# lionelblonde/sac-td3-cudagraphs-pytorch

Hardware: AMD Instinct MI355X
Metric: gradient-steps/sec (SAC, batch=256) at 1 GPU + 8-seed node; replay HBM GB/s (higher is better)
Workload: dtype f32; 1 GPU; SAC Hopper-v4 batch=256 2x256 MLP+LN, 100000 rows in a 1000000-row HBM ring, 1 critic update+Polyak per iteration, 2 actor+alpha updates every 3rd, hipGraph per 3 iterations; parallelism=1 independent seeds, one per GPU, no collective

## Files before the change

### sac-td3-cudagraphs-pytorch_amd/csrc/engine.hip

```cpp
#include <hip/hip_runtime.h>

#include <algorithm>
#include <cmath>
#include <cstdio>
#include <cstdlib>
#include <cstring>
#include <string>
#include <chrono>
#include <vector>

#include "../../include/sactd3.h"
#include "kernels.h"

static thread_local std::string g_create_error;

static inline int round_up(int x, int m) { return (x + m - 1) / m * m; }
static inline unsigned magic_div(unsigned d, unsigned long long n_max) {
  return (d > 1 && n_max * d < (1ull << 32)) ? (unsigned)(((1ull << 32) + d - 1) / d) : 0u;
}

static NetLayout make_layout(int K, int nh) {
  NetLayout L{};
  L.K = K; L.ld1 = round_up(K, 4); L.nh = nh;
  int off = 0;
// ... 68 lines not shown
  float *la = nullptr, *gscale = nullptr;
  float* ring = nullptr; float* stage_dev = nullptr;
  float *X = nullptr, *Xn = nullptr, *Xp = nullptr, *rew = nullptr, *done = nullptr;
  int* idx = nullptr;
  float *logp_n = nullptr, *logp_pi = nullptr, *logp_al = nullptr, *act_scratch = nullptr;
  float* eps[SACTD3_NUM_SITES] = {};
  float *a_z1 = nullptr, *a_xh1 = nullptr, *a_h1 = nullptr, *a_rs1 = nullptr, *a_z2 = nullptr, *a_xh2 = nullptr, *a_h2 = nullptr, *a_rs2 = nullptr, *a_tg = nullptr;
  float *a_du = nullptr, *a_dz2 = nullptr, *a_dh1 = nullptr, *a_dz1 = nullptr;
  float *qa_ps = nullptr, *qa_S = nullptr;
  float *a_ps = nullptr, *c_ps = nullptr;
  float* a_z2n = nullptr;
  float* ah_z1[4] = {}; float* ah_z2[4] = {};
  struct BatchSlot { float *X, *Xn, *rew, *done, *logp_n, *eps_c; int* idx; } bs[4] = {};
  int cur_slot = 0;
  int chain_ready = -1;
  float *c_z1 = nullptr, *c_xh1 = nullptr, *c_h1 = nullptr, *c_rs1 = nullptr, *c_z2 = nullptr, *c_dz2 = nullptr, *c_dh1 = nullptr, *c_dz1 = nullptr;
  float *t_z1 = nullptr, *t_z2 = nullptr, *q = nullptr, *qt = nullptr, *y = nullptr, *q_pi = nullptr, *dA = nullptr;
  float* s_h1 = nullptr;
  float* Gp = nullptr; int gp_slabs = 0;
  float *part = nullptr, *part_s = nullptr, *part_sa = nullptr;
  float *p_x = nullptr, *p_z1 = nullptr, *p_z2 = nullptr, *p_act = nullptr;
  float *h_obs = nullptr, *h_act = nullptr;
  int* h_done = nullptr; int predict_calls = 0;
  float* h_stage[NSTAGE] = {}; int stage_next = 0, stage_used = 0;
  float* h_batch = nullptr;

  int64_t rb_len = 0, rb_cursor = 0, qnet_updates = 0;
  hipGraphExec_t graphs[G_COUNT] = {}; int graph_nodes[G_COUNT] = {};
  std::vector<hipGraphExec_t> predict_graphs;
  hipStream_t act_stream = nullptr;
// ... 223 lines not shown
    fl += 2.0 * nets * (double)g.M * q.N * q.K;
    by += 4.0 * nets * (double)g.M * (q.N + q.K);
  }
  a.tiles_per_net = tiles;
  const int nch = (g.M + TN64_M - 1) / TN64_M;
  int S = (2 * e->num_cus + tiles * nets / 2) / (tiles * nets);
  S = std::max(1, std::min(S, std::min(e->gp_slabs, nch)));
  a.S = S;
  const long size = a.g_ns;
  {
    const dim3 grid((unsigned)(tiles * nets * S));
    char inst[96];
    snprintf(inst, sizeof(inst), "k_tn64<2,2,2,1,64>.dW(split-M x%d)", S);
    LAUNCH(inst, fl, by + 4.0 * S * nets * (double)size, TN64_KERNEL, grid, dim3(256), a);
  }
  r.Gp = e->Gp; r.S = S; r.nets = nets; r.g_ns = size; r.G = g.G;
  r.apply = g.apply; r.P = g.P; r.Mo = g.Mo; r.Vo = g.Vo; r.T = g.T; r.tau = g.tau; r.adam = g.adam; r.b1 = g.b1; r.b2 = g.b2; r.eps = g.eps;
  r.part = g.part; r.pstride = g.pstride; r.part_s = g.part_s;
  r.loss_part = g.loss_part; r.loss_n = g.loss_n; r.loss_stride = g.loss_stride; r.loss_off = g.loss_off; r.loss_scale = g.loss_scale;
  r.loss_dst = g.loss_dst; r.tick = g.tick; r.tick_extra = tick_extra;
  const dim3 grid((unsigned)((size / 4 + 255) / 256 + 4 * r.nvec + 1), (unsigned)nets);
  LAUNCH(g.apply ? (g.T ? "k_adam_red.sum+adam+polyak" : "k_adam_red.sum+adam") : "k_adam_red.sum", 0.0,
         nets * (double)size * (4.0 * S + 4.0 + (g.apply ? 24.0 : 0.0) + (g.apply && g.T ? 8.0 : 0.0)), k_adam_red, grid, dim3(256), r);
  (void)name;
  return 0;
}

static inline int tn_width(const TnProb& q) { return q.kw > 0 ? q.kw : q.ldw; }
static int launch_tn(sactd3_engine* e, hipStream_t s, const char* name, TnArgs& g, int nets, int tick_extra = 0) {
  if (g.M >= BIG_BATCH && e->Gp && !e->tune_tn_kt) {
    int tiles = 0;
    for (int i = 0; i < g.nprob; ++i) tiles += ((g.pr[i].N + TN64_N - 1) / TN64_N) * ((g.pr[i].ldw + TN64_K - 1) / TN64_K);
    if (tiles * nets >= e->tune_tn64_min) return launch_tn64(e, s, name, g, nets, tick_extra);
  }
  auto count = [&](int kt) {
    int tiles = 0;
    for (int i = 0; i < g.nprob; ++i) {
      g.pr[i].tile0 = tiles;
      tiles += ((g.pr[i].N + 15) / 16) * (((tn_width(g.pr[i]) + 15) / 16 + kt - 1) / kt);
    }
    return tiles;
  };
  int kt = (count(1) * nets > 2 * e->num_cus && g.M < BIG_BATCH) ? 2 : 1;
  if (e->tune_tn_kt) kt = e->tune_tn_kt;
// ... 9 lines not shown
  bool fold = false;
  for (int i = 0; i < g.nprob; ++i) fold = fold || g.pr[i].fold;
  char inst[96];
  snprintf(inst, sizeof(inst), fold ? "k_tn<%d,true>.%s" : "k_tn<%d>.%s", kt, name);
  g.tiles = tiles;
  if (g.pk_blocks) by += 12.0 * (g.pk.n0 + g.pk.n1);
  {
    AdamRedArgs& r = g.fin;
    r = AdamRedArgs{};
    r.s_off = -1;
    for (int i = 0; i < g.nprob; ++i) {
      const TnProb& q = g.pr[i];
      for (int f = 0; f < q.nfin; ++f) { r.vec[r.nvec].off = q.fin_off[f]; r.vec[r.nvec].slot = q.fin_slot[f]; r.vec[r.nvec].nblk = q.fin_nblk[f]; ++r.nvec; }
      if (q.fin_s_off >= 0) { r.s_off = q.fin_s_off; r.s_nblk = q.fin_s_nblk; }
    }
    r.nets = nets; r.g_ns = g.g_ns; r.G = g.G;
    r.apply = g.apply; r.P = g.P; r.Mo = g.Mo; r.Vo = g.Vo; r.T = g.T; r.tau = g.tau; r.adam = g.adam; r.b1 = g.b1; r.b2 = g.b2; r.eps = g.eps;
    r.T2 = g.T2; r.T3 = g.T3;
    r.part = g.part; r.pstride = g.pstride; r.part_s = g.part_s;
    r.loss_part = g.loss_part; r.loss_n = g.loss_n; r.loss_stride = g.loss_stride; r.loss_off = g.loss_off; r.loss_scale = g.loss_scale;
    r.loss_dst = g.loss_dst; r.tick = g.tick; r.tick_extra = tick_extra;
    g.fin_blocks = 4 * r.nvec + 1;
  }
  const dim3 grid((unsigned)((tiles + g.pk_blocks + g.fin_blocks + (nets > 1 ? 7 : 0)) & (nets > 1 ? ~7 : ~0)), 1, (unsigned)nets);
  if (!node_on(e, inst, fl, by, grid, dim3(256))) return 0;
  if (fold) {
    if (kt == 2) hipLaunchKernelGGL((k_tn<2, true>), grid, dim3(256), 0, s, g);
    else hipLaunchKernelGGL((k_tn<1, true>), grid, dim3(256), 0, s, g);
  } else if (kt == 2) hipLaunchKernelGGL(k_tn<2>, grid, dim3(256), 0, s, g);
  else hipLaunchKernelGGL(k_tn<1>, grid, dim3(256), 0, s, g);
  HIPCHK(hipGetLastError());
  return 0;
}
static TnProb tn_prob(const float* dY, int ldy, long dy_ns, int N, const float* X, int ldx, long x_ns, int K,
                      int w_off, int ldw, int b_off) {
  TnProb q{};
  q.dY = dY; q.ldy = ldy; q.dy_ns = dy_ns; q.N = N; q.X = X; q.ldx = ldx; q.x_ns = x_ns; q.K = K;
  q.w_off = w_off; q.ldw = ldw; q.b_off = b_off; q.nfin = 0; q.fin_s_off = -1;
  return q;
}
static TnProb tn_rows(const TnProb& q, int n_lo, int n) {
  TnProb r = q;
  r.dY = q.dY + n_lo; r.N = n; r.w_off = q.w_off + n_lo * q.ldw; r.b_off = q.b_off >= 0 ? q.b_off + n_lo : -1;
  if (n_lo) { r.nfin = 0; r.fin_s_off = -1; r.x_dup = 1; }
  return r;
// ... 1157 lines not shown
int sactd3_read_noise(sactd3_engine* e, int site, float* eps, int n) {
  if (!e || !eps || site < 0 || site >= SACTD3_NUM_SITES || n < 1 || n > std::max(e->B, e->maxn)) return SACTD3_EINVAL;
  USE_DEVICE(e);
  if (e->act_inflight && site == SACTD3_SITE_PREDICT) return e->fail(SACTD3_ESTATE, "read_noise: an acting call is in flight (sactd3_predict_end first)");
  HIPCHK(hipStreamSynchronize(e->stream));
  const float* src = site == SACTD3_SITE_CRITIC ? e->bs[e->cur_slot].eps_c : e->eps[site];
  HIPCHK(hipMemcpy(eps, src, sizeof(float) * (size_t)n * e->a, hipMemcpyDeviceToHost));
  return 0;
}

int sactd3_update_qnets(sactd3_engine* e) {
  if (!e) return SACTD3_EINVAL;
  USE_DEVICE(e);
  CHAIN_BREAK(e);
  e->cur_slot = 0;
  return run_graph(e, G_Q, [&](hipStream_t s) { return enqueue_update_qnets(e, s, false, nullptr); });
}
int sactd3_update_actor(sactd3_engine* e) {
  if (!e) return SACTD3_EINVAL;
  USE_DEVICE(e);
  CHAIN_BREAK(e);
  RCCHK(actor_write_begin(e));
  return run_graph(e, G_A, [&](hipStream_t s) { return enqueue_update_actor(e, s, 0); });
}
int sactd3_update_targ_nets(sactd3_engine* e, int64_t qnet_updates_so_far) {
  if (!e) return SACTD3_EINVAL;
  USE_DEVICE(e);
  CHAIN_BREAK(e);
  const bool td3 = e->cfg.prefer_td3_over_sac;
  if (td3 || qnet_updates_so_far % e->cfg.crit_targ_update_freq == 0) return enqueue_polyak(e, e->stream, true, td3);
  return 0;
}
int sactd3_step(sactd3_engine* e, int do_actor) {
  if (!e) return SACTD3_EINVAL;
  USE_DEVICE(e);
  CHAIN_BREAK(e);
  if (e->rb_len <= 0) return e->fail(SACTD3_ESTATE, "step: buffer is empty");
  const int64_t updates = e->qnet_updates + 1;
  const bool polyak = e->cfg.prefer_td3_over_sac || (updates % e->cfg.crit_targ_update_freq == 0);
  const bool act = do_actor != 0 && e->cfg.actor_update_delay > 0;
  const int which = G_STEP00 + (act ? 2 : 0) + (polyak ? 1 : 0);
  if (act) RCCHK(actor_write_begin(e));
  RCCHK(run_graph(e, which, [&](hipStream_t s) { return enqueue_step(e, s, act, polyak); }));
  e->qnet_updates = updates;
  e->cur_slot = 0;
  return 0;
}

static bool actor_dw_is_tiled64(const sactd3_engine* e) {
  if (e->B < BIG_BATCH || !e->Gp || e->tune_tn_kt) return false;
  const int tiles = ((e->nh + TN64_N - 1) / TN64_N) * ((HID + TN64_K - 1) / TN64_K) + ((HID + TN64_N - 1) / TN64_N) * ((HID + TN64_K - 1) / TN64_K)
                    + ((HID + TN64_N - 1) / TN64_N) * ((e->La.ld1 + TN64_K - 1) / TN64_K);
  return tiles >= e->tune_tn64_min;
}
static bool period_is_pipelined(const sactd3_engine* e) {
  const sactd3_config& c = e->cfg;
  if (c.actor_update_delay < 1 || c.actor_update_delay > 2 || !opening_trunk_gathers(e)) return false;
  if (c.prefer_td3_over_sac) return c.clip_norm <= 0.f && !actor_dw_is_tiled64(e);
  return c.autotune != 0;
}
static int enqueue_period(sactd3_engine* e, hipStream_t s, int variant = 0) {
  const int n = e->cfg.actor_update_delay + 1;
  if (!period_is_pipelined(e)) {
    for (int i = 0; i < n; ++i) RCCHK(enqueue_step(e, s, i == 0 && e->cfg.actor_update_delay > 0, true, i + 1 < n));
  } else {
    const int P = variant ? 3 : 0, Pnext = variant ? 0 : 3;
    RCCHK(enqueue_step(e, s, true, true, true, P, true, n - 1, Pnext, true));
    for (int i = 1; i < n; ++i) RCCHK(enqueue_step(e, s, false, true, i + 1 < n, i, true));
  }
  if (e->alpha_pending) return e->fail(SACTD3_ESTATE, "step_period: a deferred temperature step was left over");
  return 0;
}
static int enqueue_prefix(sactd3_engine* e, hipStream_t s, int variant, int m) {
  const int P = variant ? 3 : 0;
  RCCHK(enqueue_step(e, s, true, true, m > 1, P, true, m - 1, -1, true));
  for (int i = 1; i < m; ++i) RCCHK(enqueue_step(e, s, false, true, i + 1 < m, i, true));
  if (e->alpha_pending) return e->fail(SACTD3_ESTATE, "step_prefix: a deferred temperature step was left over");
  return 0;
}
static int enqueue_opening(sactd3_engine* e, hipStream_t s, int slot) {
  bool policy_done = false;
  return enqueue_update_qnets(e, s, true, nullptr, true, &policy_done, false, nullptr, slot, false, 1);
}

int sactd3_step_period(sactd3_engine* e) {
  if (!e) return SACTD3_EINVAL;
  USE_DEVICE(e);
  if (e->rb_len <= 0) return e->fail(SACTD3_ESTATE, "step_period: buffer is empty");
  const bool td3 = e->cfg.prefer_td3_over_sac;
  if (!td3 && e->cfg.crit_targ_update_freq != 1) return e->fail(SACTD3_ESTATE, "step_period: needs crit_targ_update_freq == 1");
  const int n = e->cfg.actor_update_delay + 1;
  RCCHK(actor_write_begin(e));
  if (!period_is_pipelined(e)) {
    e->chain_ready = -1;
    RCCHK(run_graph(e, G_PERIOD, [&](hipStream_t s) { return enqueue_period(e, s); }));
    e->cur_slot = 0;
  } else {
    const int v = e->chain_ready >= 0 ? e->chain_ready : 0;
    const bool have = e->chain_ready >= 0;
    e->chain_ready = -1;
    if (!have) RCCHK(run_graph(e, G_OPENING, [&](hipStream_t s) { return enqueue_opening(e, s, 0); }));
    RCCHK(run_graph(e, v ? G_PERIOD_B : G_PERIOD, [&](hipStream_t s) { return enqueue_period(e, s, v); }));
    e->chain_ready = 1 - v;
    e->cur_slot = n - 1;
  }
  e->qnet_updates += n;
  return 0;
// ... 1 lines not shown

int sactd3_step_prefix(sactd3_engine* e, int m) {
  if (!e) return SACTD3_EINVAL;
  USE_DEVICE(e);
  if (m < 1 || m > e->cfg.actor_update_delay) return e->fail(SACTD3_EINVAL, "step_prefix: 1 <= m <= actor_update_delay");
  if (e->rb_len <= 0) return e->fail(SACTD3_ESTATE, "step_prefix: buffer is empty");
  if (!e->cfg.prefer_td3_over_sac && e->cfg.crit_targ_update_freq != 1) return e->fail(SACTD3_ESTATE, "step_prefix: needs crit_targ_update_freq == 1");
  if (!period_is_pipelined(e) || m > 2) {
    for (int i = 0; i < m; ++i) RCCHK(sactd3_step(e, i == 0));
    return 0;
  }
  const int v = e->chain_ready >= 0 ? e->chain_ready : 0;
  const bool have = e->chain_ready >= 0;
  e->chain_ready = -1;
  RCCHK(actor_write_begin(e));
  if (!have) RCCHK(run_graph(e, G_OPENING, [&](hipStream_t s) { return enqueue_opening(e, s, 0); }));
  RCCHK(run_graph(e, G_PREFIX + 2 * (m - 1) + v, [&](hipStream_t s) { return enqueue_prefix(e, s, v, m); }));
  e->cur_slot = m - 1;
  e->qnet_updates += m;
  return 0;
}

int sactd3_instantiate_graphs(sactd3_engine* e) {
  if (!e) return SACTD3_EINVAL;
  USE_DEVICE(e);
  const bool same_branch = e->cfg.prefer_td3_over_sac || e->cfg.crit_targ_update_freq == 1;
  for (int act = 0; act < 2; ++act)
    for (int pol = same_branch ? 1 : 0; pol < 2; ++pol) {
      const bool a = act != 0 && e->cfg.actor_update_delay > 0, py = pol != 0;
      RCCHK(run_graph(e, G_STEP00 + (a ? 2 : 0) + (py ? 1 : 0), [&](hipStream_t s) { return enqueue_step(e, s, a, py); }, false));
// ... 171 lines not shown
      {"logp_next", S.logp_n, B}, {"logp_pi", e->logp_pi, B}, {"logp_alpha", e->logp_al, B},
      {"a_xh1", e->a_xh1, BH}, {"a_h1", e->a_h1, BH}, {"a_z2", e->a_z2, BH}, {"a_h2", e->a_h2, BH}, {"a_du", e->a_du, B * e->ldu},
      {"a_dz2", e->a_dz2, BH}, {"a_dh1", e->a_dh1, BH}, {"a_dz1", e->a_dz1, BH},
      {"c_xh1", e->c_xh1, 2 * BH}, {"c_h1", e->c_h1, 2 * BH}, {"c_z2", e->c_z2, 2 * BH}, {"c_dz2", e->c_dz2, 2 * BH},
      {"c_dh1", e->c_dh1, 2 * BH}, {"c_dz1", e->c_dz1, 2 * BH}, {"t_z2", e->t_z2, 2 * BH},
      {"q", e->q, 2 * B}, {"q_target", e->qt, 2 * B}, {"targ_q", e->y, B}, {"q_pi", e->q_pi, 2 * B}, {"dA", e->dA, 2 * B * e->a4},
  };
}
const char* sactd3_debug_names(void) {
  return "X Xn Xp rew done logp_next logp_pi logp_alpha a_xh1 a_h1 a_z2 a_h2 a_du a_dz2 a_dh1 a_dz1 c_xh1 c_h1 c_z2 c_dz2 c_dh1 c_dz1 "
         "t_z2 q q_target targ_q q_pi dA grad_actor grad_critics";
}
int64_t sactd3_debug_read(sactd3_engine* e, const char* name, float* dst, int64_t max_floats) {
  if (!e || !name) return SACTD3_EINVAL;
  USE_DEVICE(e);
  if (!strcmp(name, "grad_actor") || !strcmp(name, "grad_critics")) {
    const bool act = !strcmp(name, "grad_actor");
    const int64_t n = sactd3_param_count(e, act ? SACTD3_ACTOR : SACTD3_CRITICS);
    if (!dst) return n;
    if (max_floats < n) return e->fail(SACTD3_EINVAL, "debug_read: buffer too small");
    RCCHK(read_arena(e, act ? e->Ga : e->Gc, act ? e->La : e->Lc, act ? 1 : 2, dst));
    return n;
  }
  for (const DbgEntry& d : dbg_table(e)) {
    if (strcmp(d.name, name)) continue;
    if (!dst) return d.n;
    if (max_floats < d.n) return e->fail(SACTD3_EINVAL, "debug_read: buffer too small");
    HIPCHK(hipStreamSynchronize(e->stream));
    HIPCHK(hipMemcpy(dst, d.ptr, sizeof(float) * d.n, hipMemcpyDeviceToHost));
    return d.n;
// ... 43 lines not shown
    *usec = ms * 1000.f / (float)iters;
  }
  hipEventDestroy(t0); hipEventDestroy(t1);
  return rc;
}

int sactd3_time_nodes(sactd3_engine* e, int do_actor, int iters, int max_nodes, char* names, int names_cap,
                      float* usec, double* flops, double* bytes, int64_t* threads) {
  if (!e || iters < 1 || max_nodes < 1 || !usec) return SACTD3_EINVAL;
  USE_DEVICE(e);
  CHAIN_BREAK(e);
  if (e->rb_len <= 0) return e->fail(SACTD3_ESTATE, "time_nodes: buffer is empty");
  const bool act = do_actor != 0 && e->cfg.actor_update_delay > 0;
  const bool period = do_actor == 2 && e->cfg.actor_update_delay > 0 && (e->cfg.prefer_td3_over_sac || e->cfg.crit_targ_update_freq == 1);
  if (act || period) RCCHK(actor_write_begin(e));
  std::vector<NodeInfo> log;
  auto seq = [&]() -> int { e->node_seq = 0; return period ? enqueue_period(e, e->stream) : enqueue_step(e, e->stream, act, true); };
  auto done = [&](int rc) { e->node_only = -1; e->node_log = nullptr; e->node_seq = 0; e->node_role = ""; return rc; };
  e->node_log = &log; e->node_only = 1 << 30;
  int rc = seq();
  e->node_log = nullptr;
  if (rc != 0) return done(rc);
  const int n = (int)log.size();
  if (n > max_nodes) return done(e->fail(SACTD3_EINVAL, "time_nodes: max_nodes too small"));
  std::string joined;
  for (int k = 0; k < n; ++k) { joined += log[k].name; joined += '\n'; }
  if (names) {
    if ((int)joined.size() + 1 > names_cap) return done(e->fail(SACTD3_EINVAL, "time_nodes: names buffer too small"));
    memcpy(names, joined.c_str(), joined.size() + 1);
  }
// ... 98 lines not shown
```

### sac-td3-cudagraphs-pytorch_amd/csrc/kernels.h

```cpp
#pragma once
#include <hip/hip_runtime.h>
#include <stddef.h>
#include <stdint.h>
#include <type_traits>
#include "philox.h"

#define HID 256
#define LN_EPS 1e-5f
#define NSLOT 5
#define AS 260
#define WS 68
#define YS 20

typedef float f32x4 __attribute__((ext_vector_type(4)));

#ifdef SACTD3_STAMPS
__device__ long long g_stamps[16];
__device__ long long g_phase[8];
#define PHASE_DECL long long ph_t = 0, ph_acc[6] = {0, 0, 0, 0, 0, 0}
#define PHASE_START do { __builtin_amdgcn_s_waitcnt(0xc07f); ph_t = clock64(); } while (0)
#define PHASE(i) do { const long long n_ = clock64(); ph_acc[i] += n_ - ph_t; ph_t = n_; } while (0)
#define PHASE_DRAIN(i) do { __builtin_amdgcn_s_waitcnt(0); const long long n_ = clock64(); ph_acc[i] += n_ - ph_t; ph_t = n_; } while (0)
#define PHASE_OUT do { if (threadIdx.x == 0 && blockIdx.x == gridDim.x - 1) for (int i_ = 0; i_ < 6; ++i_) g_phase[i_] = ph_acc[i_]; } while (0)
#define STAMP(i) do { if (threadIdx.x == 0 && blockIdx.x == gridDim.x - 1 && blockIdx.y == 0 && blockIdx.z == 0) { __builtin_amdgcn_s_waitcnt(0); g_stamps[i] = clock64(); } } while (0)
// ... 96 lines not shown
  v += dpp_mov<0x141>(v);
  v += dpp_mov<0x140>(v);
  return v;
}
__device__ __forceinline__ float lane_bcast(float v, int l) {
  return __builtin_bit_cast(float, __builtin_amdgcn_readlane(__builtin_bit_cast(int, v), l));
}
__device__ __forceinline__ float wave_sum(float v) {
  v = row16_sum(v);
  return (lane_bcast(v, 0) + lane_bcast(v, 16)) + (lane_bcast(v, 32) + lane_bcast(v, 48));
}
__device__ __forceinline__ float sum4(float4 v) { return (v.x + v.y) + (v.z + v.w); }
__device__ __forceinline__ float dot4(float4 a, float4 b) { return a.x * b.x + a.y * b.y + a.z * b.z + a.w * b.w; }
__device__ __forceinline__ float4 ld4(const float* p) { return *reinterpret_cast<const float4*>(p); }
__device__ __forceinline__ void st4(float* p, float4 v) { *reinterpret_cast<float4*>(p) = v; }
__device__ __forceinline__ float4 f4(float a) { return make_float4(a, a, a, a); }
__device__ __forceinline__ float4 operator+(float4 a, float4 b) { return make_float4(a.x + b.x, a.y + b.y, a.z + b.z, a.w + b.w); }
__device__ __forceinline__ float4 operator-(float4 a, float4 b) { return make_float4(a.x - b.x, a.y - b.y, a.z - b.z, a.w - b.w); }
__device__ __forceinline__ float4 operator*(float4 a, float4 b) { return make_float4(a.x * b.x, a.y * b.y, a.z * b.z, a.w * b.w); }
__device__ __forceinline__ float4 operator*(float4 a, float b) { return make_float4(a.x * b, a.y * b, a.z * b, a.w * b); }
__device__ __forceinline__ float4 relu4(float4 a) { return make_float4(fmaxf(a.x, 0.f), fmaxf(a.y, 0.f), fmaxf(a.z, 0.f), fmaxf(a.w, 0.f)); }
__device__ __forceinline__ float4 gate4(float4 v, float4 y) {
  return make_float4(y.x > 0.f ? v.x : 0.f, y.y > 0.f ? v.y : 0.f, y.z > 0.f ? v.z : 0.f, y.w > 0.f ? v.w : 0.f);
}
__device__ __forceinline__ float4 ld4_cols(const float* row, int k, int K, int Kr, bool row_ok = true) {
  const float4 v = ld4(row + min(k, Kr - 4));
  float4 o;
  o.x = (row_ok && k < K) ? v.x : 0.f;
  o.y = (row_ok && k + 1 < K) ? v.y : 0.f;
  o.z = (row_ok && k + 2 < K) ? v.z : 0.f;
// ... 474 lines not shown
  } else {
    __syncthreads();
    if (PRO == 2) {
#pragma unroll
      for (int c = 0; c < CW; ++c) { xh[c] = av[c]; av[c] = relu4(av[c]); }
    }
  }
  STAMP(2); BLK_PH_K(1, 2);
  if (PRO != 0 && m0 + r < p.M) {
    const long ro = ni * p.act_ns + (long)(m0 + r) * HID + kb;
    const int gsz = 16 / tiles_n, g0 = tn * gsz;
#pragma unroll
    for (int c = 0; c < CW; ++c) {
      const int gc = ks * CW + c;
      if (gc >= g0 && gc < g0 + gsz) {
        if (G.xh_out) st4(G.xh_out + ro + 16 * c, xh[c]);
        if (G.h_out) st4(G.h_out + ro + 16 * c, av[c]);
      }
    }
    if (G.rstd_out && tn == 0 && ks == 0 && kq == 0) G.rstd_out[(long)ni * p.M + m0 + r] = rstd;
  }
  constexpr int NH = C4 ? 2 : 1;
  f32x4 acc[NT], ph[NT][NH];
  {
    constexpr int GC = CW < 4 ? CW : 4;
#pragma unroll
    for (int h = 0; h < NH; ++h) {
      f32x4 a0[NT], a1[NT];
#pragma unroll
      for (int nt = 0; nt < NT; ++nt) { a0[nt] = f32x4{0.f, 0.f, 0.f, 0.f}; a1[nt] = f32x4{0.f, 0.f, 0.f, 0.f}; }
#pragma unroll
      for (int c0 = h * (CW / NH); c0 < (h + 1) * (CW / NH); c0 += GC) {
// ... 37 lines not shown
            const float4 o = ld4(red + (((nt * 4 + wave + j) * NH + h) * 64 + lane) * 4);
            acc[nt][0] += o.x; acc[nt][1] += o.y; acc[nt][2] += o.z; acc[nt][3] += o.w;
          }
    }
  }
  STAMP(4); BLK_PH_K(1, 4);
  if (ks == 0) {
    float* y = G.Y + ni * p.y_ns;
#pragma unroll
    for (int nt = 0; nt < NT; ++nt) {
      const int col = n0 + 16 * nt + (lane & 15);
      if (col >= p.N) continue;
#pragma unroll
      for (int i = 0; i < 4; ++i) {
        const int row = m0 + 4 * (lane >> 4) + i;
        if (row < p.M) y[(long)row * p.ldy + col] = acc[nt][i] + bias[nt];
      }
    }
  }
  STAMP(5); BLK_PH_K(1, 5);
  BLK_MARK_K(1, 1);
}

__global__ __launch_bounds__(256) void k_nt_wide(NtArgs p) {
  __shared__ __attribute__((aligned(16))) float red[4 * 64 * 4];
  const int t = threadIdx.x, lane = t & 63, wave = t >> 6, net = blockIdx.z;
  const int r = lane & 15, kq = lane >> 4;
  if (blockIdx.x == 0 && t == 0 && net == 0) {
    if (p.tick0 || p.tick1) tick_all(p.tick0, p.tick1, p.adam_pw, p.adam_out, p.lr, p.b1, p.b2);
  }
  if (blockIdx.x == 0 && t == 64 && net == 0 && p.tick0b) tick_all(p.tick0b, nullptr, p.adam_pw_b, p.adam_out_b, p.lr_b, p.b1, p.b2);
// ... 404 lines not shown
  float* x = p.dX + net * p.dx_ns;
#pragma unroll
  for (int tt = 0; tt < TT; ++tt) {
    const int col = n0 + 16 * TT * wn + 16 * tt + r;
#pragma unroll
    for (int i = 0; i < 4; ++i) {
      const int row = m0 + 16 * wm + 4 * kq + i;
      if (row < p.M) x[(long)row * p.ldx + col] = acc[tt][i];
    }
  }
}

struct AdamRedVec { int off; int slot; int nblk; };
struct AdamRedArgs {
  const float* Gp; int S; int nets; long g_ns;
  float* G;
  int apply; float* P; float* Mo; float* Vo; float* T; float tau;
  float* T2; float* T3;
  const float* adam; float b1, b2, eps;
  AdamRedVec vec[5]; int nvec;
  const float* part; int pstride;
  int s_off; int s_nblk; const float* part_s;
  const float* loss_part; int loss_n, loss_stride, loss_off; float loss_scale; float* loss_dst; int* tick;
  int tick_extra;
};
__device__ __forceinline__ void adam_red_commit(const AdamRedArgs& a, long off, float4 g, float4 w, float4 m, float4 v, float4 tt, float step, float sq2) {
  st4(a.G + off, g);
  if (a.apply) {
    const float omb1 = 1.0f - a.b1, omb2 = 1.0f - a.b2;
    m = m + (g - m) * omb1;
    v = v * a.b2 + g * g * omb2;
    w.x -= step * (m.x / (sqrtf(v.x) / sq2 + a.eps)); w.y -= step * (m.y / (sqrtf(v.y) / sq2 + a.eps));
    w.z -= step * (m.z / (sqrtf(v.z) / sq2 + a.eps)); w.w -= step * (m.w / (sqrtf(v.w) / sq2 + a.eps));
    st4(a.Mo + off, m); st4(a.Vo + off, v); st4(a.P + off, w);
    if (a.T) {
      const float4 t1 = tt + (w - tt) * a.tau;
      st4(a.T + off, t1);
      if (a.T2) {
        const float4 t2 = t1 + (w - t1) * a.tau;
        st4(a.T2 + off, t2);
        if (a.T3) st4(a.T3 + off, t2 + (w - t2) * a.tau);
      }
    }
  }
}
__device__ __forceinline__ void adam_red_tail_body(const AdamRedArgs& a, int rel, int net) {
  const int t = threadIdx.x;
  const float step = a.apply ? a.adam[0] : 0.f, sq2 = a.apply ? a.adam[1] : 1.f;
  if (rel < 4 * a.nvec) {
    const int e = rel >> 2, quarter = rel & 3;
    int voff = a.vec[0].off, vslot = a.vec[0].slot, nb = a.vec[0].nblk;
    if (e == 1) { voff = a.vec[1].off; vslot = a.vec[1].slot; nb = a.vec[1].nblk; }
    if (e == 2) { voff = a.vec[2].off; vslot = a.vec[2].slot; nb = a.vec[2].nblk; }
    if (e == 3) { voff = a.vec[3].off; vslot = a.vec[3].slot; nb = a.vec[3].nblk; }
    if (e == 4) { voff = a.vec[4].off; vslot = a.vec[4].slot; nb = a.vec[4].nblk; }
    const int c4 = (t >> 4) + 16 * quarter, sub = t & 15;
    const long off = net * a.g_ns + voff + 4 * c4;
    float4 w = f4(0.f), m = f4(0.f), v = f4(0.f), tt = f4(0.f);
    if (a.apply && sub == 0) { w = ld4(a.P + off); m = ld4(a.Mo + off); v = ld4(a.Vo + off); if (a.T) tt = ld4(a.T + off); }
    const float* pp = a.part + ((long)net * a.pstride * NSLOT + vslot) * HID + 4 * c4;
    float4 g = f4(0.f);
    for (int blk = sub; blk < nb; blk += 64) {
      const float4 v0 = ld4(pp + (long)blk * NSLOT * HID), v1 = ld4(pp + (long)min(blk + 16, nb - 1) * NSLOT * HID);
      const float4 v2 = ld4(pp + (long)min(blk + 32, nb - 1) * NSLOT * HID), v3 = ld4(pp + (long)min(blk + 48, nb - 1) * NSLOT * HID);
      g = g + v0;
      if (blk + 16 < nb) g = g + v1;
      if (blk + 32 < nb) g = g + v2;
      if (blk + 48 < nb) g = g + v3;
    }
    g.x = row16_sum(g.x); g.y = row16_sum(g.y); g.z = row16_sum(g.z); g.w = row16_sum(g.w);
    if (sub == 0) adam_red_commit(a, off, g, w, m, v, tt, step, sq2);
    return;
  }
  if (t >= 64) return;
  const bool extras = net == 0;
  float loss_acc = 0.f; int tick_v = 0;
  if (extras) {
    if (a.loss_dst) for (int k = t; k < a.loss_n; k += 64) loss_acc += a.loss_part[(long)k * a.loss_stride + a.loss_off];
    if (t == 0 && a.tick) tick_v = *a.tick;
  }
  if (a.s_off >= 0) {
    const long off = net * a.g_ns + a.s_off;
    float4 w = f4(0.f), m = f4(0.f), v = f4(0.f), tt = f4(0.f);
    if (a.apply && t == 0) { w = ld4(a.P + off); m = ld4(a.Mo + off); v = ld4(a.Vo + off); if (a.T) tt = ld4(a.T + off); }
    float sg = 0.f;
    for (int blk = t; blk < a.s_nblk; blk += 64) sg += a.part_s[((long)net * a.pstride + blk) * 2];
    sg = wave_sum(sg);
    if (t == 0) adam_red_commit(a, off, make_float4(sg, 0.f, 0.f, 0.f), w, m, v, tt, step, sq2);
  }
  if (extras) {
    if (a.loss_dst) {
      const float sl = wave_sum(loss_acc);
      if (t == 0) *a.loss_dst = sl * a.loss_scale;
    }
    if (t == 0 && a.tick) *a.tick = tick_v + 1 + a.tick_extra;
  }
}

struct PolyakArgs { float* t0; const float* p0; long n0; float* t1; const float* p1; long n1; float tau; };
__device__ __forceinline__ void polyak_body(const PolyakArgs& a, unsigned block, unsigned nblocks) {
  const long n = a.n0 + a.n1;
  for (long i = ((long)block * 256 + threadIdx.x) * 4; i < n; i += (long)nblocks * 1024) {
    float* t = i < a.n0 ? a.t0 + i : a.t1 + (i - a.n0);
// ... 11 lines not shown
  int nfin; int fin_slot[3]; int fin_off[3]; int fin_nblk[3];
  int fin_s_off; int fin_s_nblk;
  int tile0;
  int xr;
  int x_dup;
  int xr_force;
  int kw;
  int fold, f_ln, f_g_off, f_be_off;
  const float* f_xh; const float* f_rstd; const float* f_ps; float* f_dz;
  const float* f_g;
};
constexpr int PS_W = 32;
struct TnArgs {
  TnProb pr[4]; int nprob; int M;
  float* G; long g_ns;
  int apply; float* P; float* Mo; float* Vo; float* T; float tau; float* T2; float* T3;
  const float* adam;
  float b1, b2, eps;
  const float* part; int pstride; const float* part_s;
  const float* loss_part; int loss_n, loss_stride, loss_off; float loss_scale; float* loss_dst; int* tick;
  int tiles; int pk_blocks; PolyakArgs pk;
  int fin_blocks; AdamRedArgs fin;
};

struct AdamState { float w, m, v, t; };
__device__ __forceinline__ AdamState adam_fetch(const TnArgs& p, long off) {
  AdamState s{0.f, 0.f, 0.f, 0.f};
  if (p.apply) { s.w = p.P[off]; s.m = p.Mo[off]; s.v = p.Vo[off]; if (p.T) s.t = p.T[off]; }
  return s;
}
__device__ __forceinline__ void adam_commit(const TnArgs& p, long off, float g, AdamState s, float step, float sq2) {
  p.G[off] = g;
  if (p.apply) {
    const float m = s.m + (g - s.m) * (1.0f - p.b1);
    const float v = s.v * p.b2 + g * g * (1.0f - p.b2);
    const float w = s.w - step * (m / (sqrtf(v) / sq2 + p.eps));
    p.Mo[off] = m; p.Vo[off] = v; p.P[off] = w;
    if (p.T) {
      const float t1 = s.t + (w - s.t) * p.tau;
      p.T[off] = t1;
      if (p.T2) {
        const float t2 = t1 + (w - t1) * p.tau;
        p.T2[off] = t2;
        if (p.T3) p.T3[off] = t2 + (w - t2) * p.tau;
      }
    }
  }
}

template <int KT, bool FOLD = false>
__global__ __launch_bounds__(256) void k_tn(TnArgs p) {
  __shared__ __attribute__((aligned(16))) float red[KT * 4 * 64 * 4];
  __shared__ __attribute__((aligned(16))) float Ys[256 * YS];
  __shared__ __attribute__((aligned(16))) float Xs[KT * 256 * YS];
  __shared__ float cred[16 * 17];
  __shared__ __attribute__((aligned(16))) float fsum[FOLD ? 16 * 4 * 8 : 4];
  const int t = threadIdx.x, lane = t & 63, wave = t >> 6, net = blockIdx.z;
  const int r = lane & 15, kq = lane >> 4;
  BLK_MARK(0);
  if ((int)blockIdx.x >= p.tiles) {
    const int x = (int)blockIdx.x - p.tiles;
    if (x < p.pk_blocks) { if (net == 0) polyak_body(p.pk, x, p.pk_blocks); }
    else if (x - p.pk_blocks < p.fin_blocks) adam_red_tail_body(p.fin, x - p.pk_blocks, net);
    BLK_MARK(1);
    return;
  }
  int pi = 0;
  if (p.nprob > 1 && (int)blockIdx.x >= p.pr[1].tile0) pi = 1;
  if (p.nprob > 2 && (int)blockIdx.x >= p.pr[2].tile0) pi = 2;
  if (p.nprob > 3 && (int)blockIdx.x >= p.pr[3].tile0) pi = 3;
  const TnProb q = p.pr[pi];
  const int local = blockIdx.x - q.tile0;
  const int kw = q.kw > 0 ? q.kw : q.ldw;
  const int tiles_k = (((kw + 15) >> 4) + KT - 1) / KT;
  int tn, tk;
  xcd_tile(local, (q.N + 15) >> 4, tiles_k, q.xr, tn, tk);
  const int n0 = tn * 16, k0 = tk * 16 * KT;
  const long nbase = net * p.g_ns;
// ... 96 lines not shown
  STAMP(2); BLK_PH(2);
#pragma unroll
  for (int kt = 0; kt < KT; ++kt) st4(red + ((kt * 4 + wave) * 64 + lane) * 4, make_float4(acc[kt][0], acc[kt][1], acc[kt][2], acc[kt][3]));
  if (want_bias) cred[fpart * 17 + fcol] = asum;
  if (fold_vec) {
    float v[8] = {cg.x, cg.y, cg.z, cg.w, cb.x, cb.y, cb.z, cb.w};
#pragma unroll
    for (int j = 0; j < 8; ++j) { v[j] += dpp_mov<0x124>(v[j]); v[j] += dpp_mov<0x128>(v[j]); }
    if ((lane & 15) < 4) {
      float* d = fsum + ((wave * 4 + (lane >> 4)) * 4 + (lane & 3)) * 8;
      st4(d, make_float4(v[0], v[1], v[2], v[3])); st4(d + 4, make_float4(v[4], v[5], v[6], v[7]));
    }
  }
  __syncthreads();
  STAMP(3); BLK_PH(3);
  if (wave < KT && ecol < kw) {
    const float* rr = red + (wave * 4 * 64 + lane) * 4;
    const float4 a = ld4(rr), b = ld4(rr + 256), c = ld4(rr + 512), d = ld4(rr + 768);
    const float o[4] = {(a.x + b.x) + (c.x + d.x), (a.y + b.y) + (c.y + d.y), (a.z + b.z) + (c.z + d.z), (a.w + b.w) + (c.w + d.w)};
#pragma unroll
    for (int i = 0; i < 4; ++i) {
      const int row = n0 + 4 * (lane >> 4) + i;
      if (row < q.N) adam_commit(p, nbase + q.w_off + (long)row * q.ldw + ecol, ecol < q.K ? o[i] : 0.f, st[i], step, sq2);
    }
  }
  if (foff >= 0) {
    float v = 0.f;
    if (lane < 16) {
#pragma unroll
      for (int i = 0; i < 16; ++i) v += cred[i * 17 + fcol];
    } else {
      const float* f = fsum + (fcol >> 2) * 8 + (lane < 32 ? 0 : 4) + (fcol & 3);
#pragma unroll
      for (int i = 0; i < 16; ++i) v += f[i * 32];
    }
    adam_commit(p, foff, v, fstate, step, sq2);
  }
  STAMP(4); BLK_PH(4);
  BLK_MARK(1);
}

struct Tn64Prob {
  const float* dY; int ldy; long dy_ns; int N;
  const float* X; int ldx; long x_ns; int K;
  int w_off, ldw, b_off;
  int tiles_n, tiles_k, tile0;
};
struct Tn64Args {
  Tn64Prob pr[3]; int nprob; int M; int nets; int S;
  int tiles_per_net;
  float* Gp; long g_ns;
// ... 162 lines not shown
  }
  if (want_bias) {
    constexpr int PARTS = 256 / TN;
    csum[t] = asum;
    __syncthreads();
    if (t < TN && n0 + t < q.N) {
      float v = 0.f;
#pragma unroll
      for (int i = 0; i < PARTS; ++i) v += csum[i * TN + t];
      Gs[q.b_off + n0 + t] = v;
    }
  }
  STAMP(3);
}

__global__ __launch_bounds__(256) void k_adam_red(AdamRedArgs a) {
  const int net = blockIdx.y, t = threadIdx.x;
  const int main_blocks = (int)((a.g_ns / 4 + 255) / 256);
  const int bx = blockIdx.x;
  if (bx >= main_blocks) { adam_red_tail_body(a, bx - main_blocks, net); return; }
  const float step = a.apply ? a.adam[0] : 0.f, sq2 = a.apply ? a.adam[1] : 1.f;
  const long i = ((long)bx * 256 + t) * 4;
  bool mine = i < a.g_ns && !(a.s_off >= 0 && i == a.s_off);
#pragma unroll
  for (int e = 0; e < 5; ++e)
    if (e < a.nvec && i >= a.vec[e].off && i < a.vec[e].off + HID) mine = false;
  if (mine) {
    const long off = net * a.g_ns + i;
    float4 w = f4(0.f), m = f4(0.f), v = f4(0.f), tt = f4(0.f);
    if (a.apply) { w = ld4(a.P + off); m = ld4(a.Mo + off); v = ld4(a.Vo + off); if (a.T) tt = ld4(a.T + off); }
    float4 gs[8];
#pragma unroll
    for (int sl = 0; sl < 8; ++sl) gs[sl] = ld4(a.Gp + ((long)min(sl, a.S - 1) * a.nets + net) * a.g_ns + i);
    float4 g = gs[0];
#pragma unroll
    for (int sl = 1; sl < 8; ++sl) if (sl < a.S) g = g + gs[sl];
    adam_red_commit(a, off, g, w, m, v, tt, step, sq2);
  }
}

struct ActorTail {
  const float* z2;
  const float* P; NetLayout L;
  int B, o, a, ln, sac, mode, train;
  const DevCtl* ctl; const int* ctr; int site_buf; unsigned site_code;
  float* eps;
  const float* scale; const float* bias; const float* min_ac; const float* max_ac;
  float* dst; int ldd; int dst_off;
  const float* obs_src; int lds;
  float* logp;
  float* h2; float* xh2; float* rstd2; float* tg;
  int a4;
// ... 546 lines not shown
  Row16 dy, vals[3];
#pragma unroll
  for (int q = 0; q < 4; ++q) dy.v[q] = gate4(wo.v[q] * dq, y.v[q]);
  const Row16 dz = ln_bwd(dy, xh, rstd, go, p.ln);
#pragma unroll
  for (int q = 0; q < 4; ++q) { vals[0].v[q] = dy.v[q] * xh.v[q]; vals[1].v[q] = dy.v[q]; vals[2].v[q] = h.v[q] * dq; }
#pragma unroll
  for (int nt = 0; nt < NT; ++nt)
#pragma unroll
    for (int c = 0; c < 4; ++c) { PIN(bv[nt][c].x); PIN(bv[nt][c].y); PIN(bv[nt][c].z); PIN(bv[nt][c].w); }
  row_st(Dz + row * AS, sub, dz);
#pragma unroll
  for (int q = 0; q < 4; ++q) {
    const int col = 4 * sub + 64 * q;
    if (col >= c_lo && col < c_lo + CB) {
      if (valid) st4(p.dz2 + ((long)net * p.B + b) * HID + col, dz.v[q]);
#pragma unroll
      for (int sl = 0; sl < 3; ++sl) st4(cs + (sl * 16 + row) * CB + (col - c_lo), vals[sl].v[q]);
    }
  }
  if (tk == 0 && sub == 0) {
    sc[row][0] = dq; sc[row][1] = err * err;
    if (valid) {
      p.q[(long)net * p.B + b] = qv;
      if (net == 0) { p.qt[b] = qt0; p.qt[p.B + b] = qt1; p.y[b] = yv; }
    }
  }
  __syncthreads();
  const long blk = (long)net * p.pstride + tm;
  if (t < 3 * CB) {
    const int sl = t / CB, c = t - sl * CB;
// ... 648 lines not shown
  row_pin(w[7]); add_n(dpp_mov<0x157>(d), w[7]);
#pragma unroll
  for (int c = 0; c < 4; ++c) { PIN(bv[c].x); PIN(bv[c].y); PIN(bv[c].z); PIN(bv[c].w); }
  if (tk == 0 && valid && sub < nh) p.du[(long)b * p.ldu + sub] = d;
  Row16 dy, vals[2];
#pragma unroll
  for (int q = 0; q < 4; ++q) dy.v[q] = gate4(dh.v[q], hh.v[q]);
  const Row16 dz = ln_bwd(dy, xh, rstd, g, p.ln);
#pragma unroll
  for (int q = 0; q < 4; ++q) { vals[0].v[q] = dy.v[q] * xh.v[q]; vals[1].v[q] = dy.v[q]; }
  row_st(Dz + row * AS, sub, dz);
#pragma unroll
  for (int q = 0; q < 4; ++q) {
    const int col = 4 * sub + 64 * q;
    if (col >= c_lo && col < c_lo + CB) {
      if (valid) st4(p.dz2 + (long)b * HID + col, dz.v[q]);
#pragma unroll
      for (int sl = 0; sl < 2; ++sl) st4(cs + (sl * 16 + row) * CB + (col - c_lo), vals[sl].v[q]);
    }
  }
  __syncthreads();
  if (t < 2 * CB) {
    const int sl = t / CB, c = t - sl * CB;
    float sum = 0.f;
#pragma unroll
    for (int i = 0; i < 16; ++i) sum += cs[(sl * 16 + i) * CB + c];
    p.part[((long)tm * NSLOT + sl) * HID + c_lo + c] = sum;
  }
  f32x4 acc = {0.f, 0.f, 0.f, 0.f};
#pragma unroll
  for (int c = 0; c < 4; ++c) { const float4 av = ld4(Dz + r * AS + nb + 16 * c); MFMA4(acc, av, bv[c]); }
// ... 63 lines not shown
```

Baseline: 18820 gradient-steps/s.

## Skip gradient buffer stores in period graphs and add write-through store policy

In period and prefix graphs with no gradient clipping, the weight-gradient kernels are built with KEEP_G=false. They apply Adam straight from the reduced gradient and skip writing the full gradient array to HBM. The change also drops the f_dz stores and tracks which gradient buffers are stale, so debug reads of them now fail. Separately, it adds buffer stores with a cache-policy flag (write-through or streaming) for layer-1 activations, which are on by default, plus optional flags for z2 and dz2, meant to cut cache pollution from producer writes. The cost is more kernel template instantiations and a new failure path for debug reads of gradient buffers.

```diff
diff --git a/sac-td3-cudagraphs-pytorch_amd/csrc/engine.hip b/sac-td3-cudagraphs-pytorch_amd/csrc/engine.hip
--- a/sac-td3-cudagraphs-pytorch_amd/csrc/engine.hip
+++ b/sac-td3-cudagraphs-pytorch_amd/csrc/engine.hip
@@ -106,6 +106,7 @@
   struct BatchSlot { float *X, *Xn, *rew, *done, *logp_n, *eps_c; int* idx; } bs[4] = {};
   int cur_slot = 0;
   int chain_ready = -1;
+  bool lean_stores = false, grads_stale[2] = {false, false};
   float *c_z1 = nullptr, *c_xh1 = nullptr, *c_h1 = nullptr, *c_rs1 = nullptr, *c_z2 = nullptr, *c_dz2 = nullptr, *c_dh1 = nullptr, *c_dz1 = nullptr;
   float *t_z1 = nullptr, *t_z2 = nullptr, *q = nullptr, *qt = nullptr, *y = nullptr, *q_pi = nullptr, *dA = nullptr;
   float* s_h1 = nullptr;
@@ -359,20 +360,24 @@
     snprintf(inst, sizeof(inst), "k_tn64<2,2,2,1,64>.dW(split-M x%d)", S);
     LAUNCH(inst, fl, by + 4.0 * S * nets * (double)size, TN64_KERNEL, grid, dim3(256), a);
   }
-  r.Gp = e->Gp; r.S = S; r.nets = nets; r.g_ns = size; r.G = g.G;
+  r.Gp = e->Gp; r.S = S; r.nets = nets; r.g_ns = size; r.G = g.G; r.keep_g = !(e->lean_stores && g.apply);
   r.apply = g.apply; r.P = g.P; r.Mo = g.Mo; r.Vo = g.Vo; r.T = g.T; r.tau = g.tau; r.adam = g.adam; r.b1 = g.b1; r.b2 = g.b2; r.eps = g.eps;
   r.part = g.part; r.pstride = g.pstride; r.part_s = g.part_s;
   r.loss_part = g.loss_part; r.loss_n = g.loss_n; r.loss_stride = g.loss_stride; r.loss_off = g.loss_off; r.loss_scale = g.loss_scale;
   r.loss_dst = g.loss_dst; r.tick = g.tick; r.tick_extra = tick_extra;
   const dim3 grid((unsigned)((size / 4 + 255) / 256 + 4 * r.nvec + 1), (unsigned)nets);
-  LAUNCH(g.apply ? (g.T ? "k_adam_red.sum+adam+polyak" : "k_adam_red.sum+adam") : "k_adam_red.sum", 0.0,
-         nets * (double)size * (4.0 * S + 4.0 + (g.apply ? 24.0 : 0.0) + (g.apply && g.T ? 8.0 : 0.0)), k_adam_red, grid, dim3(256), r);
+  const char* rname = g.apply ? (g.T ? "k_adam_red.sum+adam+polyak" : "k_adam_red.sum+adam") : "k_adam_red.sum";
+  const double rbytes = nets * (double)size * (4.0 * S + 4.0 + (g.apply ? 24.0 : 0.0) + (g.apply && g.T ? 8.0 : 0.0));
+  if (r.keep_g) LAUNCH(rname, 0.0, rbytes, k_adam_red<true>, grid, dim3(256), r);
+  else LAUNCH(rname, 0.0, rbytes, k_adam_red<false>, grid, dim3(256), r);
   (void)name;
   return 0;
 }
 
 static inline int tn_width(const TnProb& q) { return q.kw > 0 ? q.kw : q.ldw; }
 static int launch_tn(sactd3_engine* e, hipStream_t s, const char* name, TnArgs& g, int nets, int tick_extra = 0) {
+  g.keep_g = !(e->lean_stores && g.apply);
+  if (!g.keep_g) for (int i = 0; i < g.nprob; ++i) g.pr[i].f_dz = nullptr;
   if (g.M >= BIG_BATCH && e->Gp && !e->tune_tn_kt) {
     int tiles = 0;
     for (int i = 0; i < g.nprob; ++i) tiles += ((g.pr[i].N + TN64_N - 1) / TN64_N) * ((g.pr[i].ldw + TN64_K - 1) / TN64_K);
@@ -412,7 +417,7 @@
       for (int f = 0; f < q.nfin; ++f) { r.vec[r.nvec].off = q.fin_off[f]; r.vec[r.nvec].slot = q.fin_slot[f]; r.vec[r.nvec].nblk = q.fin_nblk[f]; ++r.nvec; }
       if (q.fin_s_off >= 0) { r.s_off = q.fin_s_off; r.s_nblk = q.fin_s_nblk; }
     }
-    r.nets = nets; r.g_ns = g.g_ns; r.G = g.G;
+    r.nets = nets; r.g_ns = g.g_ns; r.G = g.G; r.keep_g = g.keep_g;
     r.apply = g.apply; r.P = g.P; r.Mo = g.Mo; r.Vo = g.Vo; r.T = g.T; r.tau = g.tau; r.adam = g.adam; r.b1 = g.b1; r.b2 = g.b2; r.eps = g.eps;
     r.T2 = g.T2; r.T3 = g.T3;
     r.part = g.part; r.pstride = g.pstride; r.part_s = g.part_s;
@@ -422,11 +427,17 @@
   }
   const dim3 grid((unsigned)((tiles + g.pk_blocks + g.fin_blocks + (nets > 1 ? 7 : 0)) & (nets > 1 ? ~7 : ~0)), 1, (unsigned)nets);
   if (!node_on(e, inst, fl, by, grid, dim3(256))) return 0;
-  if (fold) {
-    if (kt == 2) hipLaunchKernelGGL((k_tn<2, true>), grid, dim3(256), 0, s, g);
-    else hipLaunchKernelGGL((k_tn<1, true>), grid, dim3(256), 0, s, g);
-  } else if (kt == 2) hipLaunchKernelGGL(k_tn<2>, grid, dim3(256), 0, s, g);
-  else hipLaunchKernelGGL(k_tn<1>, grid, dim3(256), 0, s, g);
+  if (g.keep_g) {
+    if (fold) {
+      if (kt == 2) hipLaunchKernelGGL((k_tn<2, true>), grid, dim3(256), 0, s, g);
+      else hipLaunchKernelGGL((k_tn<1, true>), grid, dim3(256), 0, s, g);
+    } else if (kt == 2) hipLaunchKernelGGL(k_tn<2>, grid, dim3(256), 0, s, g);
+    else hipLaunchKernelGGL(k_tn<1>, grid, dim3(256), 0, s, g);
+  } else if (fold) {
+    if (kt == 2) hipLaunchKernelGGL((k_tn<2, true, false>), grid, dim3(256), 0, s, g);
+    else hipLaunchKernelGGL((k_tn<1, true, false>), grid, dim3(256), 0, s, g);
+  } else if (kt == 2) hipLaunchKernelGGL((k_tn<2, false, false>), grid, dim3(256), 0, s, g);
+  else hipLaunchKernelGGL((k_tn<1, false, false>), grid, dim3(256), 0, s, g);
   HIPCHK(hipGetLastError());
   return 0;
 }
@@ -1614,14 +1625,18 @@
   USE_DEVICE(e);
   CHAIN_BREAK(e);
   e->cur_slot = 0;
-  return run_graph(e, G_Q, [&](hipStream_t s) { return enqueue_update_qnets(e, s, false, nullptr); });
+  RCCHK(run_graph(e, G_Q, [&](hipStream_t s) { return enqueue_update_qnets(e, s, false, nullptr); }));
+  e->grads_stale[0] = false;
+  return 0;
 }
 int sactd3_update_actor(sactd3_engine* e) {
   if (!e) return SACTD3_EINVAL;
   USE_DEVICE(e);
   CHAIN_BREAK(e);
   RCCHK(actor_write_begin(e));
-  return run_graph(e, G_A, [&](hipStream_t s) { return enqueue_update_actor(e, s, 0); });
+  RCCHK(run_graph(e, G_A, [&](hipStream_t s) { return enqueue_update_actor(e, s, 0); }));
+  e->grads_stale[1] = false;
+  return 0;
 }
 int sactd3_update_targ_nets(sactd3_engine* e, int64_t qnet_updates_so_far) {
   if (!e) return SACTD3_EINVAL;
@@ -1644,6 +1659,8 @@
   RCCHK(run_graph(e, which, [&](hipStream_t s) { return enqueue_step(e, s, act, polyak); }));
   e->qnet_updates = updates;
   e->cur_slot = 0;
+  e->grads_stale[0] = false;
+  if (act) e->grads_stale[1] = false;
   return 0;
 }
 
@@ -1659,8 +1676,19 @@
   if (c.prefer_td3_over_sac) return c.clip_norm <= 0.f && !actor_dw_is_tiled64(e);
   return c.autotune != 0;
 }
+struct LeanStores {
+  sactd3_engine* e;
+  explicit LeanStores(sactd3_engine* e_) : e(e_) { e->lean_stores = e->cfg.clip_norm <= 0.f; }
+  ~LeanStores() { e->lean_stores = false; }
+};
+static void mark_grads_stale(sactd3_engine* e) {
+  if (e->cfg.clip_norm > 0.f) return;
+  e->grads_stale[0] = true;
+  if (e->cfg.actor_update_delay > 0) e->grads_stale[1] = true;
+}
 static int enqueue_period(sactd3_engine* e, hipStream_t s, int variant = 0) {
   const int n = e->cfg.actor_update_delay + 1;
+  LeanStores lean(e);
   if (!period_is_pipelined(e)) {
     for (int i = 0; i < n; ++i) RCCHK(enqueue_step(e, s, i == 0 && e->cfg.actor_update_delay > 0, true, i + 1 < n));
   } else {
@@ -1673,6 +1701,7 @@
 }
 static int enqueue_prefix(sactd3_engine* e, hipStream_t s, int variant, int m) {
   const int P = variant ? 3 : 0;
+  LeanStores lean(e);
   RCCHK(enqueue_step(e, s, true, true, m > 1, P, true, m - 1, -1, true));
   for (int i = 1; i < m; ++i) RCCHK(enqueue_step(e, s, false, true, i + 1 < m, i, true));
   if (e->alpha_pending) return e->fail(SACTD3_ESTATE, "step_prefix: a deferred temperature step was left over");
@@ -1691,6 +1720,7 @@
   if (!td3 && e->cfg.crit_targ_update_freq != 1) return e->fail(SACTD3_ESTATE, "step_period: needs crit_targ_update_freq == 1");
   const int n = e->cfg.actor_update_delay + 1;
   RCCHK(actor_write_begin(e));
+  mark_grads_stale(e);
   if (!period_is_pipelined(e)) {
     e->chain_ready = -1;
     RCCHK(run_graph(e, G_PERIOD, [&](hipStream_t s) { return enqueue_period(e, s); }));
@@ -1722,6 +1752,7 @@
   const bool have = e->chain_ready >= 0;
   e->chain_ready = -1;
   RCCHK(actor_write_begin(e));
+  mark_grads_stale(e);
   if (!have) RCCHK(run_graph(e, G_OPENING, [&](hipStream_t s) { return enqueue_opening(e, s, 0); }));
   RCCHK(run_graph(e, G_PREFIX + 2 * (m - 1) + v, [&](hipStream_t s) { return enqueue_prefix(e, s, v, m); }));
   e->cur_slot = m - 1;
@@ -1923,6 +1954,8 @@
 int64_t sactd3_debug_read(sactd3_engine* e, const char* name, float* dst, int64_t max_floats) {
   if (!e || !name) return SACTD3_EINVAL;
   USE_DEVICE(e);
+  if (((!strcmp(name, "grad_critics") || !strcmp(name, "c_dz1")) && e->grads_stale[0]) || ((!strcmp(name, "grad_actor") || !strcmp(name, "a_dz1")) && e->grads_stale[1]))
+    return e->fail(SACTD3_ESTATE, "debug_read: period graphs do not store this buffer; run an API-path update or sactd3_step first");
   if (!strcmp(name, "grad_actor") || !strcmp(name, "grad_critics")) {
     const bool act = !strcmp(name, "grad_actor");
     const int64_t n = sactd3_param_count(e, act ? SACTD3_ACTOR : SACTD3_CRITICS);
@@ -1996,6 +2029,7 @@
   const bool act = do_actor != 0 && e->cfg.actor_update_delay > 0;
   const bool period = do_actor == 2 && e->cfg.actor_update_delay > 0 && (e->cfg.prefer_td3_over_sac || e->cfg.crit_targ_update_freq == 1);
   if (act || period) RCCHK(actor_write_begin(e));
+  if (period) mark_grads_stale(e);
   std::vector<NodeInfo> log;
   auto seq = [&]() -> int { e->node_seq = 0; return period ? enqueue_period(e, e->stream) : enqueue_step(e, e->stream, act, true); };
   auto done = [&](int rc) { e->node_only = -1; e->node_log = nullptr; e->node_seq = 0; e->node_role = ""; return rc; };
diff --git a/sac-td3-cudagraphs-pytorch_amd/csrc/kernels.h b/sac-td3-cudagraphs-pytorch_amd/csrc/kernels.h
--- a/sac-td3-cudagraphs-pytorch_amd/csrc/kernels.h
+++ b/sac-td3-cudagraphs-pytorch_amd/csrc/kernels.h
@@ -134,6 +134,20 @@
 __device__ __forceinline__ float dot4(float4 a, float4 b) { return a.x * b.x + a.y * b.y + a.z * b.z + a.w * b.w; }
 __device__ __forceinline__ float4 ld4(const float* p) { return *reinterpret_cast<const float4*>(p); }
 __device__ __forceinline__ void st4(float* p, float4 v) { *reinterpret_cast<float4*>(p) = v; }
+#ifndef SACTD3_WT
+#define SACTD3_WT 1
+#endif
+constexpr bool WT_ACT1 = (SACTD3_WT & 1) != 0;
+constexpr bool WT_Z2 = (SACTD3_WT & 2) != 0;
+constexpr bool WT_DZ = (SACTD3_WT & 4) != 0;
+typedef unsigned int u32x4 __attribute__((ext_vector_type(4)));
+__device__ __forceinline__ void st4_wt(float* base, long off, float4 v) {
+  const u32x4 u = {__float_as_uint(v.x), __float_as_uint(v.y), __float_as_uint(v.z), __float_as_uint(v.w)};
+  __builtin_amdgcn_raw_buffer_store_b128(u, __builtin_amdgcn_make_buffer_rsrc(base, 0, 0x7fffffff, 0x00020000), (int)(4 * off), 0, 16);
+}
+__device__ __forceinline__ void st1_wt(float* p, float v) { __hip_atomic_store(p, v, __ATOMIC_RELAXED, __HIP_MEMORY_SCOPE_AGENT); }
+template <bool WT> __device__ __forceinline__ void st4_pol(float* base, long off, float4 v) { if (WT) st4_wt(base, off, v); else st4(base + off, v); }
+template <bool WT> __device__ __forceinline__ void st1_pol(float* p, float v) { if (WT) st1_wt(p, v); else *p = v; }
 __device__ __forceinline__ float4 f4(float a) { return make_float4(a, a, a, a); }
 __device__ __forceinline__ float4 operator+(float4 a, float4 b) { return make_float4(a.x + b.x, a.y + b.y, a.z + b.z, a.w + b.w); }
 __device__ __forceinline__ float4 operator-(float4 a, float4 b) { return make_float4(a.x - b.x, a.y - b.y, a.z - b.z, a.w - b.w); }
@@ -638,8 +652,8 @@
     for (int c = 0; c < CW; ++c) {
       const int gc = ks * CW + c;
       if (gc >= g0 && gc < g0 + gsz) {
-        if (G.xh_out) st4(G.xh_out + ro + 16 * c, xh[c]);
-        if (G.h_out) st4(G.h_out + ro + 16 * c, av[c]);
+        if (G.xh_out) st4_pol<WT_ACT1>(G.xh_out, ro + 16 * c, xh[c]);
+        if (G.h_out) st4_pol<WT_ACT1>(G.h_out, ro + 16 * c, av[c]);
       }
     }
     if (G.rstd_out && tn == 0 && ks == 0 && kq == 0) G.rstd_out[(long)ni * p.M + m0 + r] = rstd;
@@ -707,7 +721,7 @@
 #pragma unroll
       for (int i = 0; i < 4; ++i) {
         const int row = m0 + 4 * (lane >> 4) + i;
-        if (row < p.M) y[(long)row * p.ldy + col] = acc[nt][i] + bias[nt];
+        if (row < p.M) st1_pol<WT_Z2>(y + (long)row * p.ldy + col, acc[nt][i] + bias[nt]);
       }
     }
   }
@@ -1142,7 +1156,7 @@
 struct AdamRedVec { int off; int slot; int nblk; };
 struct AdamRedArgs {
   const float* Gp; int S; int nets; long g_ns;
-  float* G;
+  float* G; int keep_g;
   int apply; float* P; float* Mo; float* Vo; float* T; float tau;
   float* T2; float* T3;
   const float* adam; float b1, b2, eps;
@@ -1152,8 +1166,9 @@
   const float* loss_part; int loss_n, loss_stride, loss_off; float loss_scale; float* loss_dst; int* tick;
   int tick_extra;
 };
+template <bool KEEP_G>
 __device__ __forceinline__ void adam_red_commit(const AdamRedArgs& a, long off, float4 g, float4 w, float4 m, float4 v, float4 tt, float step, float sq2) {
-  st4(a.G + off, g);
+  if (KEEP_G) st4(a.G + off, g);
   if (a.apply) {
     const float omb1 = 1.0f - a.b1, omb2 = 1.0f - a.b2;
     m = m + (g - m) * omb1;
@@ -1172,6 +1187,7 @@
     }
   }
 }
+template <bool KEEP_G>
 __device__ __forceinline__ void adam_red_tail_body(const AdamRedArgs& a, int rel, int net) {
   const int t = threadIdx.x;
   const float step = a.apply ? a.adam[0] : 0.f, sq2 = a.apply ? a.adam[1] : 1.f;
@@ -1197,7 +1213,7 @@
       if (blk + 48 < nb) g = g + v3;
     }
     g.x = row16_sum(g.x); g.y = row16_sum(g.y); g.z = row16_sum(g.z); g.w = row16_sum(g.w);
-    if (sub == 0) adam_red_commit(a, off, g, w, m, v, tt, step, sq2);
+    if (sub == 0) adam_red_commit<KEEP_G>(a, off, g, w, m, v, tt, step, sq2);
     return;
   }
   if (t >= 64) return;
@@ -1214,7 +1230,7 @@
     float sg = 0.f;
     for (int blk = t; blk < a.s_nblk; blk += 64) sg += a.part_s[((long)net * a.pstride + blk) * 2];
     sg = wave_sum(sg);
-    if (t == 0) adam_red_commit(a, off, make_float4(sg, 0.f, 0.f, 0.f), w, m, v, tt, step, sq2);
+    if (t == 0) adam_red_commit<KEEP_G>(a, off, make_float4(sg, 0.f, 0.f, 0.f), w, m, v, tt, step, sq2);
   }
   if (extras) {
     if (a.loss_dst) {
@@ -1256,6 +1272,7 @@
 struct TnArgs {
   TnProb pr[4]; int nprob; int M;
   float* G; long g_ns;
+  int keep_g;
   int apply; float* P; float* Mo; float* Vo; float* T; float tau; float* T2; float* T3;
   const float* adam;
   float b1, b2, eps;
@@ -1271,8 +1288,9 @@
   if (p.apply) { s.w = p.P[off]; s.m = p.Mo[off]; s.v = p.Vo[off]; if (p.T) s.t = p.T[off]; }
   return s;
 }
+template <bool KEEP_G>
 __device__ __forceinline__ void adam_commit(const TnArgs& p, long off, float g, AdamState s, float step, float sq2) {
-  p.G[off] = g;
+  if (KEEP_G) p.G[off] = g;
   if (p.apply) {
     const float m = s.m + (g - s.m) * (1.0f - p.b1);
     const float v = s.v * p.b2 + g * g * (1.0f - p.b2);
@@ -1290,7 +1308,7 @@
   }
 }
 
-template <int KT, bool FOLD = false>
+template <int KT, bool FOLD = false, bool KEEP_G = true>
 __global__ __launch_bounds__(256) void k_tn(TnArgs p) {
   __shared__ __attribute__((aligned(16))) float red[KT * 4 * 64 * 4];
   __shared__ __attribute__((aligned(16))) float Ys[256 * YS];
@@ -1303,7 +1321,7 @@
   if ((int)blockIdx.x >= p.tiles) {
     const int x = (int)blockIdx.x - p.tiles;
     if (x < p.pk_blocks) { if (net == 0) polyak_body(p.pk, x, p.pk_blocks); }
-    else if (x - p.pk_blocks < p.fin_blocks) adam_red_tail_body(p.fin, x - p.pk_blocks, net);
+    else if (x - p.pk_blocks < p.fin_blocks) adam_red_tail_body<KEEP_G>(p.fin, x - p.pk_blocks, net);
     BLK_MARK(1);
     return;
   }
@@ -1430,6 +1448,11 @@
   }
   __syncthreads();
   STAMP(3); BLK_PH(3);
+  if (!KEEP_G) {
+#pragma unroll
+    for (int i = 0; i < 4; ++i) { PIN(st[i].w); PIN(st[i].m); PIN(st[i].v); PIN(st[i].t); }
+    PIN(fstate.w); PIN(fstate.m); PIN(fstate.v); PIN(fstate.t);
+  }
   if (wave < KT && ecol < kw) {
     const float* rr = red + (wave * 4 * 64 + lane) * 4;
     const float4 a = ld4(rr), b = ld4(rr + 256), c = ld4(rr + 512), d = ld4(rr + 768);
@@ -1437,7 +1460,7 @@
 #pragma unroll
     for (int i = 0; i < 4; ++i) {
       const int row = n0 + 4 * (lane >> 4) + i;
-      if (row < q.N) adam_commit(p, nbase + q.w_off + (long)row * q.ldw + ecol, ecol < q.K ? o[i] : 0.f, st[i], step, sq2);
+      if (row < q.N) adam_commit<KEEP_G>(p, nbase + q.w_off + (long)row * q.ldw + ecol, ecol < q.K ? o[i] : 0.f, st[i], step, sq2);
     }
   }
   if (foff >= 0) {
@@ -1450,7 +1473,7 @@
 #pragma unroll
       for (int i = 0; i < 16; ++i) v += f[i * 32];
     }
-    adam_commit(p, foff, v, fstate, step, sq2);
+    adam_commit<KEEP_G>(p, foff, v, fstate, step, sq2);
   }
   STAMP(4); BLK_PH(4);
   BLK_MARK(1);
@@ -1643,11 +1666,12 @@
   STAMP(3);
 }
 
+template <bool KEEP_G = true>
 __global__ __launch_bounds__(256) void k_adam_red(AdamRedArgs a) {
   const int net = blockIdx.y, t = threadIdx.x;
   const int main_blocks = (int)((a.g_ns / 4 + 255) / 256);
   const int bx = blockIdx.x;
-  if (bx >= main_blocks) { adam_red_tail_body(a, bx - main_blocks, net); return; }
+  if (bx >= main_blocks) { adam_red_tail_body<KEEP_G>(a, bx - main_blocks, net); return; }
   const float step = a.apply ? a.adam[0] : 0.f, sq2 = a.apply ? a.adam[1] : 1.f;
   const long i = ((long)bx * 256 + t) * 4;
   bool mine = i < a.g_ns && !(a.s_off >= 0 && i == a.s_off);
@@ -1664,7 +1688,7 @@
     float4 g = gs[0];
 #pragma unroll
     for (int sl = 1; sl < 8; ++sl) if (sl < a.S) g = g + gs[sl];
-    adam_red_commit(a, off, g, w, m, v, tt, step, sq2);
+    adam_red_commit<KEEP_G>(a, off, g, w, m, v, tt, step, sq2);
   }
 }
 
@@ -2241,7 +2265,7 @@
   for (int q = 0; q < 4; ++q) {
     const int col = 4 * sub + 64 * q;
     if (col >= c_lo && col < c_lo + CB) {
-      if (valid) st4(p.dz2 + ((long)net * p.B + b) * HID + col, dz.v[q]);
+      if (valid) st4_pol<WT_DZ>(p.dz2, ((long)net * p.B + b) * HID + col, dz.v[q]);
 #pragma unroll
       for (int sl = 0; sl < 3; ++sl) st4(cs + (sl * 16 + row) * CB + (col - c_lo), vals[sl].v[q]);
     }
@@ -2920,7 +2944,7 @@
   for (int q = 0; q < 4; ++q) {
     const int col = 4 * sub + 64 * q;
     if (col >= c_lo && col < c_lo + CB) {
-      if (valid) st4(p.dz2 + (long)b * HID + col, dz.v[q]);
+      if (valid) st4_pol<WT_DZ>(p.dz2, (long)b * HID + col, dz.v[q]);
 #pragma unroll
       for (int sl = 0; sl < 2; ++sl) st4(cs + (sl * 16 + row) * CB + (col - c_lo), vals[sl].v[q]);
     }
```

Measured after the change: 19490 gradient-steps/s (median of 6 runs). 1.04x the previous value.
